# bentotten/radiation_ppo

Measured on AMD Instinct MI355X. Metric: env steps/sec (whole node) at 4096 envs; PPO iters/sec at 1/2/4/8 GPUs, higher is better.
Workload: dtype f32 policy / f64+int32 env

## Files before the change

radiation_ppo_amd/csrc/rs_ppo_grad2.hpp:

```cpp
#pragma once
#include "rs_mlp.hpp"

#define RS_T2 33

#ifdef RS_K7_STAMPS
#define RS_K7_NPH 16
__device__ unsigned long long rs_k7_stamp_table[2][RS_K7_NPH];
#define RS_STAMP_ENTRY const unsigned long long st_rt0 = __builtin_amdgcn_s_memrealtime(); const unsigned long long st_t0 = rs_k7_now();
#define RS_STAMP_DECL unsigned long long st_acc[RS_K7_NPH] = {0}; unsigned long long st_last = rs_k7_now(); st_acc[12] = st_last - st_t0;
#define RS_STAMP_EXIT(net) do { RS_STAMP(13); if ((threadIdx.x & 63) == 0) { st_acc[14] = __builtin_amdgcn_s_memrealtime() - st_rt0; \
                           for (int q = 0; q < RS_K7_NPH; ++q) atomicAdd(&rs_k7_stamp_table[net][q], st_acc[q]); } } while (0)
#define RS_STAMP(i) do { __builtin_amdgcn_sched_barrier(0); asm volatile("; RS_STAMP_MARK " #i); const unsigned long long t_ = rs_k7_now(); st_acc[i] += t_ - st_last; st_last = t_; \
                         __builtin_amdgcn_sched_barrier(0); } while (0)
__device__ __forceinline__ unsigned long long rs_k7_now() {
    unsigned long long t;
    asm volatile("s_memtime %0\n\ts_waitcnt lgkmcnt(0)" : "=s"(t) :: "memory");
    return t;
}
#else
#define RS_STAMP_ENTRY
#define RS_STAMP_DECL
#define RS_STAMP_EXIT(net)
#ifdef RS_K7_NO_PHASE_FENCE
#define RS_STAMP(i) do {} while (0)
#else
#define RS_STAMP(i) __builtin_amdgcn_sched_barrier(0)
#endif
#endif
#define RS_XRAW 400
#define RS_XSC 192
#define RS_G2_WAVE_FLOATS ((64 + 32) * RS_T2 + RS_XRAW + RS_XSC + 64)

__host__ __device__ constexpr int rs_grad2_lds_floats(int nout) {
    return ((rs_mlp_lds_floats(nout) + 3) & ~3) + 2 * 2 * 16 * 64 + 2 * 4 * 64 + 8 * RS_G2_WAVE_FLOATS;
}

__device__ __forceinline__ float rs_other_half(float x, int h) {
    const auto r = __builtin_amdgcn_permlane32_swap(__float_as_uint(x), __float_as_uint(x), false, false);
    return __uint_as_float(h ? r[0] : r[1]);
}

__device__ __forceinline__ void rs_stage32(float* T, const f32x16& v, int c, int h) {
#pragma unroll
    for (int r = 0; r < 16; ++r) T[rs_kappa(r, h) * RS_T2 + c] = v[r];
}

template <int NOUT>
__device__ __forceinline__ void rs_ppo_grad2_body(const RsMlpParams prm, const rs_ppo_batch B, float* partial,
                                                  double* stat_partial, const int* stop,
                                                  const rs_update_state* ust, int* snap,
                                                  const int bid, const int nblocks) {
    extern __shared__ __align__(16) float smem_f[];
    if (snap && bid == 0 && threadIdx.x == 0) { snap[0] = ust->adam_step; snap[1] = ust->stopped; }
    if (stop && *stop) return;
    RS_STAMP_ENTRY
    RsMlpLds<NOUT> W;
    W.carve(smem_f);
    float* w2tf = smem_f + ((rs_mlp_lds_floats(NOUT) + 3) & ~3);
    float* w3tf = w2tf + 2 * 2 * 16 * 64;
    const int wid = __builtin_amdgcn_readfirstlane(threadIdx.x >> 6);
    const int lane = threadIdx.x & 63, h = lane >> 5, c = lane & 31;
    const int l15 = lane & 15, l4 = lane >> 4;
    float* Qt = w3tf + 2 * 4 * 64 + wid * RS_G2_WAVE_FLOATS;
    float* Pt = Qt + 64 * RS_T2;
    float* xraw = Pt + 32 * RS_T2;
    float* xsc = xraw + RS_XRAW;
    float* dbl = xsc + RS_XSC;
    float* w1b = W.w1f;
    for (int i = threadIdx.x; i < 2 * 6 * 64; i += blockDim.x) {
        const int l = i & 63, s = (i >> 6) % 6, it = i / (6 * 64);
        const int row = 32 * it + (l & 31), k = 2 * s + (l >> 5);
        w1b[i] = RS_TANH_PRESCALE * ((k < RS_IN) ? prm.w1[row * RS_IN + k] : prm.b1[row]);
    }
    for (int i = threadIdx.x; i < 2 * 2 * 16 * 64; i += blockDim.x) {
        const int ri = i & 3, l = (i >> 2) & 63, r4 = (i >> 8) & 3, kt = (i >> 10) & 1, it = i >> 11;
        const int r = 4 * r4 + ri;
        w2tf[i] = prm.w2[(32 * kt + rs_kappa(r, l >> 5)) * RS_HID + 32 * it + (l & 31)];
        W.w2f[i] = RS_TANH_PRESCALE * prm.w2[(32 * it + (l & 31)) * RS_HID + 32 * kt + rs_kappa(r, l >> 5)];
    }
    for (int i = threadIdx.x; i < 2 * 4 * 64; i += blockDim.x) {
        int l = i & 63, sq = (i >> 6) & 3, it = i >> 8;
        int o = 2 * sq + (l >> 5);
        w3tf[i] = (o < NOUT) ? prm.w3[o * RS_HID + 32 * it + (l & 31)] : 0.0f;
    }
    for (int i = threadIdx.x; i < 2 * NOUT * 32; i += blockDim.x) {
        int q = i & 31, o = (i >> 5) % NOUT, hh = i / (32 * NOUT);
        if constexpr (NOUT == 8) { q = 4 * (i >> 6) + (i & 3); o = (i >> 2) & 7; hh = (i >> 5) & 1; }
        W.w3h[i] = prm.w3[o * RS_HID + 32 * (q >> 4) + rs_kappa(q & 15, hh)];
    }
    for (int i = threadIdx.x; i < 64; i += blockDim.x) W.b2[i] = RS_TANH_PRESCALE * prm.b2[i];
    for (int i = threadIdx.x; i < NOUT; i += blockDim.x) W.b3[i] = prm.b3[i];
    dbl[lane] = 0.0f;
    __syncthreads();

    const int M = B.M;
    const int groups = (M + 31) / 32;
    const int wave_g = bid * 8 + wid, n_waves = nblocks * 8;

    f32x16 acc2[2][2];
    f32x4 acc1[4], acc3[4];
#pragma unroll
    for (int a = 0; a < 2; ++a)
#pragma unroll
        for (int r = 0; r < 16; ++r) { acc2[a][0][r] = 0.f; acc2[a][1][r] = 0.f; }
#pragma unroll
    for (int a = 0; a < 4; ++a)
#pragma unroll
        for (int r = 0; r < 4; ++r) { acc1[a][r] = 0.f; acc3[a][r] = 0.f; }
    f32x4 accs;
#pragma unroll
    for (int r = 0; r < 4; ++r) accs[r] = 0.f;

    const int trips = (groups + n_waves - 1) / n_waves;
    const long x_last = (long)M * RS_IN - 1;
    auto dma_rows = [&](int g) {
        const char* gx = reinterpret_cast<const char*>(B.x + (long)g * (32 * RS_IN));
        const int lim = (int)(x_last - (long)g * (32 * RS_IN));
#pragma unroll
        for (int i = 0; i < 6; ++i) {
            const int o = min(i * 64 + lane, lim);
            __builtin_amdgcn_global_load_lds((const __attribute__((address_space(1))) void*)(gx + 4u * (unsigned)o),
                                             (__attribute__((address_space(3))) void*)(xraw + i * 64), 4, 0, 0);
        }
    };
    auto dma_scal = [&](int g) {
        const int m0 = g * 32;
        const int ms = min(m0 + c, M - 1);
        if constexpr (NOUT == 8) {
            const int mi = min(m0 + (lane >> 1), M - 1);
            const int* src = reinterpret_cast<const int*>(B.act) + 2 * (size_t)mi + (lane & 1);
            __builtin_amdgcn_global_load_lds((const __attribute__((address_space(1))) void*)src,
                                             (__attribute__((address_space(3))) void*)(xsc), 4, 0, 0);
        }
        if constexpr (NOUT == 8) {
            const float* src = (h ? B.logp_old : B.adv) + ms;
            __builtin_amdgcn_global_load_lds((const __attribute__((address_space(1))) void*)src,
                                             (__attribute__((address_space(3))) void*)(xsc + 64), 4, 0, 0);
        }
        {
            const float* src = (h ? B.ret : B.w) + ms;
            __builtin_amdgcn_global_load_lds((const __attribute__((address_space(1))) void*)src,
                                             (__attribute__((address_space(3))) void*)(xsc + 128), 4, 0, 0);
        }
    };
    {
        const int g0 = wave_g < groups ? wave_g : groups - 1;
        dma_rows(g0);
        dma_scal(g0);
    }
    float w3v[NOUT == 1 ? 32 : 1], db2r[2] = {0.0f, 0.0f};
    if constexpr (NOUT == 1) {
        const float4* wrow = reinterpret_cast<const float4*>(W.w3h + h * 32);
#pragma unroll
        for (int b = 0; b < 8; ++b) {
            const float4 t = wrow[b];
            w3v[4 * b + 0] = t.x; w3v[4 * b + 1] = t.y; w3v[4 * b + 2] = t.z; w3v[4 * b + 3] = t.w;
        }
    }
    RS_STAMP_DECL
    for (int trip = 0; trip < trips; ++trip) {
        RS_STAMP(15);
        const int gi_raw = wave_g + trip * n_waves;
        const int gi = gi_raw < groups ? gi_raw : groups - 1;
        const int m = gi * 32 + c;
        const bool valid = gi_raw < groups && m < M;
        asm volatile("s_waitcnt vmcnt(0)" ::: "memory");
#if defined(RS_K7_ALIGN) && RS_K7_ALIGN >= 1
        __builtin_amdgcn_s_barrier();
#endif
        const float wi = valid ? xsc[128 + c] : 0.0f;
        const int s_act = reinterpret_cast<const int*>(xsc)[2 * c];
        const float s_adv = xsc[64 + c], s_lpo = xsc[96 + c], s_ret = xsc[160 + c];
        float xv[6];
#pragma unroll
        for (int s6 = 0; s6 < 6; ++s6) xv[s6] = xraw[c * RS_IN + 2 * s6 + h];
        if (h) xv[5] = 1.0f;
        RS_STAMP(0);
        f32x16 H1[2], H2[2];
#pragma unroll
        for (int it = 0; it < 2; ++it)
#pragma unroll
            for (int r = 0; r < 16; ++r) H1[it][r] = 0.0f;
        {
            float a0 = w1b[(0 * 6 + 0) * 64 + lane], a1 = w1b[(1 * 6 + 0) * 64 + lane];
#pragma unroll
            for (int s = 0; s < 6; ++s) {
                const float b = xv[s];
                float n0 = 0.f, n1 = 0.f;
                if (s + 1 < 6) { n0 = w1b[(0 * 6 + s + 1) * 64 + lane]; n1 = w1b[(1 * 6 + s + 1) * 64 + lane]; }
                H1[0] = __builtin_amdgcn_mfma_f32_32x32x2f32(a0, b, H1[0], 0, 0, 0);
                H1[1] = __builtin_amdgcn_mfma_f32_32x32x2f32(a1, b, H1[1], 0, 0, 0);
                a0 = n0; a1 = n1;
            }
        }
        RS_STAMP(1);
#pragma unroll
        for (int it = 0; it < 2; ++it)
#pragma unroll
            for (int r = 0; r < 16; ++r) H1[it][r] = rs_tanh_scaled(H1[it][r]);
#pragma unroll
        for (int it = 0; it < 2; ++it)
#pragma unroll
            for (int q = 0; q < 4; ++q) {
                const float4 b = *reinterpret_cast<const float4*>(W.b2 + 32 * it + 8 * q + 4 * h);
                H2[it][4 * q + 0] = b.x; H2[it][4 * q + 1] = b.y; H2[it][4 * q + 2] = b.z; H2[it][4 * q + 3] = b.w;
            }
        RS_STAMP(2);
        {
            const float4* wq = reinterpret_cast<const float4*>(W.w2f) + lane;
            float4 a0 = wq[0], a1 = wq[(1 * 2 + 0) * 4 * 64];
#pragma unroll
            for (int g4 = 0; g4 < 8; ++g4) {
                const int kt = g4 >> 2, r0 = 4 * (g4 & 3);
                float4 n0 = a0, n1 = a1;
                if (g4 + 1 < 8) {
                    n0 = wq[((0 * 2 + ((g4 + 1) >> 2)) * 4 + ((g4 + 1) & 3)) * 64];
                    n1 = wq[((1 * 2 + ((g4 + 1) >> 2)) * 4 + ((g4 + 1) & 3)) * 64];
                }
                H2[0] = __builtin_amdgcn_mfma_f32_32x32x2f32(a0.x, H1[kt][r0 + 0], H2[0], 0, 0, 0);
                H2[1] = __builtin_amdgcn_mfma_f32_32x32x2f32(a1.x, H1[kt][r0 + 0], H2[1], 0, 0, 0);
                H2[0] = __builtin_amdgcn_mfma_f32_32x32x2f32(a0.y, H1[kt][r0 + 1], H2[0], 0, 0, 0);
                H2[1] = __builtin_amdgcn_mfma_f32_32x32x2f32(a1.y, H1[kt][r0 + 1], H2[1], 0, 0, 0);
                H2[0] = __builtin_amdgcn_mfma_f32_32x32x2f32(a0.z, H1[kt][r0 + 2], H2[0], 0, 0, 0);
                H2[1] = __builtin_amdgcn_mfma_f32_32x32x2f32(a1.z, H1[kt][r0 + 2], H2[1], 0, 0, 0);
                H2[0] = __builtin_amdgcn_mfma_f32_32x32x2f32(a0.w, H1[kt][r0 + 3], H2[0], 0, 0, 0);
                H2[1] = __builtin_amdgcn_mfma_f32_32x32x2f32(a1.w, H1[kt][r0 + 3], H2[1], 0, 0, 0);
                a0 = n0; a1 = n1;
            }
        }
        rs_stage32(Qt, H1[0], c, h);
        rs_stage32(Qt + 32 * RS_T2, H1[1], c, h);
        RS_STAMP(3);
#if defined(RS_K7_ALIGN) && RS_K7_ALIGN >= 2
        __builtin_amdgcn_s_barrier();
#endif
#pragma unroll
        for (int it = 0; it < 2; ++it)
#pragma unroll
            for (int r = 0; r < 16; ++r) H2[it][r] = rs_tanh_scaled(H2[it][r]);
        RS_STAMP(4);
        float out[NOUT];
        if constexpr (NOUT == 1) {
            float pacc = 0.0f;
#pragma unroll
            for (int q = 0; q < 32; ++q) pacc = fmaf(w3v[q], H2[q >> 4][q & 15], pacc);
            const float q = rs_other_half(pacc, h);
            out[0] = (h ? (q + pacc) : (pacc + q)) + W.b3[0];
        } else {
            f32x4 pacc[2];
#pragma unroll
            for (int r = 0; r < 4; ++r) { pacc[0][r] = 0.0f; pacc[1][r] = 0.0f; }
            const float4* wrow = reinterpret_cast<const float4*>(W.w3h) + 8 * h + (lane & 3);
            float4 wv[8][2];
#pragma unroll
            for (int b = 0; b < 8; ++b) { wv[b][0] = wrow[16 * b]; wv[b][1] = wrow[16 * b + 4]; }
#pragma unroll
            for (int b = 0; b < 8; ++b) {
                const int kt = b >> 2, r4 = b & 3;
                pacc[0] = __builtin_amdgcn_mfma_f32_4x4x1f32(wv[b][0].x, H2[kt][4 * r4 + 0], pacc[0], 0, 0, 0);
                pacc[1] = __builtin_amdgcn_mfma_f32_4x4x1f32(wv[b][1].x, H2[kt][4 * r4 + 0], pacc[1], 0, 0, 0);
                pacc[0] = __builtin_amdgcn_mfma_f32_4x4x1f32(wv[b][0].y, H2[kt][4 * r4 + 1], pacc[0], 0, 0, 0);
                pacc[1] = __builtin_amdgcn_mfma_f32_4x4x1f32(wv[b][1].y, H2[kt][4 * r4 + 1], pacc[1], 0, 0, 0);
                pacc[0] = __builtin_amdgcn_mfma_f32_4x4x1f32(wv[b][0].z, H2[kt][4 * r4 + 2], pacc[0], 0, 0, 0);
                pacc[1] = __builtin_amdgcn_mfma_f32_4x4x1f32(wv[b][1].z, H2[kt][4 * r4 + 2], pacc[1], 0, 0, 0);
                pacc[0] = __builtin_amdgcn_mfma_f32_4x4x1f32(wv[b][0].w, H2[kt][4 * r4 + 3], pacc[0], 0, 0, 0);
                pacc[1] = __builtin_amdgcn_mfma_f32_4x4x1f32(wv[b][1].w, H2[kt][4 * r4 + 3], pacc[1], 0, 0, 0);
            }
#pragma unroll
            for (int o = 0; o < NOUT; ++o) {
                const float p = pacc[o >> 2][o & 3];
                const float q = rs_other_half(p, h);
                out[o] = (h ? (q + p) : (p + q)) + W.b3[o];
            }
        }
        RS_STAMP(5);
        float dz[NOUT], sq[4];
        if (NOUT == 8) {
            const int a = s_act;
            const float adv = s_adv, lpo = s_lpo;
            float mx = out[0];
#pragma unroll
            for (int j = 1; j < NOUT; ++j) mx = fmaxf(mx, out[j]);
            float se = 0.f;
#pragma unroll
            for (int j = 0; j < NOUT; ++j) se += __expf(out[j] - mx);
            const float lse = __logf(se);
            float lp[NOUT], pj[NOUT], ent = 0.f, logp = 0.f;
#pragma unroll
            for (int j = 0; j < NOUT; ++j) {
                lp[j] = (out[j] - mx) - lse;
                pj[j] = __expf(lp[j]);
                ent -= pj[j] * lp[j];
                logp = (a == j) ? lp[j] : logp;
            }
            const float ratio = __expf(logp - lpo);
            const float lo = 1.0f - B.clip_ratio, hi = 1.0f + B.clip_ratio;
            const float clipped = fminf(fmaxf(ratio, lo), hi);
            const float s1 = ratio * adv, s2 = clipped * adv;
            const float surr = fminf(s1, s2);
            const bool inside = ratio >= lo && ratio <= hi;
            const float dr = (inside || s1 < s2) ? adv : 0.0f;
            const float g_lp = -wi * dr * ratio;
#pragma unroll
            for (int j = 0; j < NOUT; ++j) dz[j] = g_lp * (((a == j) ? 1.0f : 0.0f) - pj[j]);
            sq[0] = wi * (lpo - logp);
            sq[1] = wi * ent;
            sq[2] = wi * ((ratio > hi || ratio < lo) ? 1.0f : 0.0f);
            sq[3] = wi * surr;
        } else {
            const float diff = out[0] - s_ret;
            dz[0] = 2.0f * B.vf_coef * wi * diff;
            sq[0] = wi * diff * diff; sq[1] = 0.f; sq[2] = 0.f; sq[3] = 0.f;
        }
        RS_STAMP(6);

        float* Dz = xraw;
        if constexpr (NOUT == 1) {
            constexpr int T4 = 36;
            float* zrow = xraw + 96;
            float* ones = xraw + 160;
            zrow[32 * h + c] = h ? sq[0] : dz[0];
            ones[c] = 1.0f;
            float4 av[8];
#pragma unroll
            for (int hf = 0; hf < 2; ++hf) {
                rs_wave_sync();
#pragma unroll
                for (int r = 0; r < 16; ++r) Pt[rs_kappa(r, h) * T4 + c] = H2[hf][r];
                rs_wave_sync();
                if (hf == 0) {
#pragma unroll
                    for (int q = 0; q < 8; ++q) av[q] = *reinterpret_cast<const float4*>(zrow + 32 * (lane & 1) + 4 * q);
                }
                const float* brow = (hf == 0 && h) ? ones : Pt + c * T4;
                float4 bv[8];
#pragma unroll
                for (int q = 0; q < 8; ++q) bv[q] = *reinterpret_cast<const float4*>(brow + 4 * q);
#pragma unroll
                for (int q = 0; q < 8; ++q) {
                    acc3[hf] = __builtin_amdgcn_mfma_f32_4x4x1f32(av[q].x, bv[q].x, acc3[hf], 0, 0, 0);
                    acc3[hf] = __builtin_amdgcn_mfma_f32_4x4x1f32(av[q].y, bv[q].y, acc3[hf], 0, 0, 0);
                    acc3[hf] = __builtin_amdgcn_mfma_f32_4x4x1f32(av[q].z, bv[q].z, acc3[hf], 0, 0, 0);
                    acc3[hf] = __builtin_amdgcn_mfma_f32_4x4x1f32(av[q].w, bv[q].w, acc3[hf], 0, 0, 0);
                }
            }
        } else {
        if (h == 0) {
#pragma unroll
            for (int o = 0; o < NOUT; ++o) Dz[o * RS_T2 + c] = dz[o];
        } else {
#pragma unroll
            for (int q = 0; q < 4; ++q) Dz[(8 + q) * RS_T2 + c] = sq[q];
        }
#pragma unroll
        for (int hf = 0; hf < 2; ++hf) {
            rs_wave_sync();
            rs_stage32(Pt, H2[hf], c, h);
            rs_wave_sync();
            const bool a_row = l15 < NOUT || (l15 >= 8 && l15 < 12);
            float a_c = a_row ? Dz[l15 * RS_T2 + l4] : 0.0f;
            float b_c[2];
#pragma unroll
            for (int u = 0; u < 2; ++u) b_c[u] = Pt[(16 * u + l15) * RS_T2 + l4];
#pragma unroll
            for (int s = 0; s < 8; ++s) {
                float a_n = 0.f, b_n[2] = {0.f, 0.f};
                if (s + 1 < 8) {
                    a_n = a_row ? Dz[l15 * RS_T2 + 4 * (s + 1) + l4] : 0.0f;
#pragma unroll
                    for (int u = 0; u < 2; ++u) b_n[u] = Pt[(16 * u + l15) * RS_T2 + 4 * (s + 1) + l4];
                }
                const float a_dz = (l15 < NOUT) ? a_c : 0.0f;
#pragma unroll
                for (int u = 0; u < 2; ++u) acc3[2 * hf + u] = __builtin_amdgcn_mfma_f32_16x16x4f32(a_dz, b_c[u], acc3[2 * hf + u], 0, 0, 0);
                if (hf == 0) accs = __builtin_amdgcn_mfma_f32_16x16x4f32(a_c, 1.0f, accs, 0, 0, 0);
                a_c = a_n;
#pragma unroll
                for (int u = 0; u < 2; ++u) b_c[u] = b_n[u];
            }
        }
        }
        RS_STAMP(7);
        if (NOUT == 8) {
#pragma unroll
            for (int it = 0; it < 2; ++it) {
                f32x16 t;
#pragma unroll
                for (int r = 0; r < 16; ++r) t[r] = 0.f;
#pragma unroll
                for (int s = 0; s < 4; ++s) {
                    const float b = h ? dz[(2 * s + 1) % NOUT] : dz[(2 * s) % NOUT];
                    t = __builtin_amdgcn_mfma_f32_32x32x2f32(w3tf[(it * 4 + s) * 64 + lane], b, t, 0, 0, 0);
                }
#pragma unroll
                for (int r = 0; r < 16; ++r) { const float hv = H2[it][r]; H2[it][r] = fmaf(-(t[r] * hv), hv, t[r]); }
            }
        } else {
#pragma unroll
            for (int kt = 0; kt < 2; ++kt)
#pragma unroll
                for (int r = 0; r < 16; ++r) {
                    const float hv = H2[kt][r];
                    const float d = w3v[kt * 16 + r] * dz[0];
                    H2[kt][r] = fmaf(-(d * hv), hv, d);
                }
        }
        {
            const int gn_raw = wave_g + (trip + 1) * n_waves;
            const int gn = gn_raw < groups ? gn_raw : groups - 1;
            asm volatile("s_waitcnt lgkmcnt(0)" ::: "memory");
            dma_rows(gn);
            dma_scal(gn);
        }
        RS_STAMP(8);
#if defined(RS_K7_ALIGN) && RS_K7_ALIGN >= 3
        __builtin_amdgcn_s_barrier();
#endif
        rs_wave_sync();
        rs_stage32(Pt, H2[0], c, h);
        f32x16 D1[2];
#pragma unroll
        for (int it = 0; it < 2; ++it)
#pragma unroll
            for (int r = 0; r < 16; ++r) D1[it][r] = 0.f;
        {
            const float4* wq = reinterpret_cast<const float4*>(w2tf) + lane;
            float4 a0 = wq[0], a1 = wq[(1 * 2 + 0) * 4 * 64];
#pragma unroll
            for (int g4 = 0; g4 < 8; ++g4) {
                const int kt = g4 >> 2, r0 = 4 * (g4 & 3);
                float4 n0 = a0, n1 = a1;
                if (g4 + 1 < 8) {
                    n0 = wq[((0 * 2 + ((g4 + 1) >> 2)) * 4 + ((g4 + 1) & 3)) * 64];
                    n1 = wq[((1 * 2 + ((g4 + 1) >> 2)) * 4 + ((g4 + 1) & 3)) * 64];
                }
                D1[0] = __builtin_amdgcn_mfma_f32_32x32x2f32(a0.x, H2[kt][r0 + 0], D1[0], 0, 0, 0);
                D1[1] = __builtin_amdgcn_mfma_f32_32x32x2f32(a1.x, H2[kt][r0 + 0], D1[1], 0, 0, 0);
                D1[0] = __builtin_amdgcn_mfma_f32_32x32x2f32(a0.y, H2[kt][r0 + 1], D1[0], 0, 0, 0);
                D1[1] = __builtin_amdgcn_mfma_f32_32x32x2f32(a1.y, H2[kt][r0 + 1], D1[1], 0, 0, 0);
                D1[0] = __builtin_amdgcn_mfma_f32_32x32x2f32(a0.z, H2[kt][r0 + 2], D1[0], 0, 0, 0);
                D1[1] = __builtin_amdgcn_mfma_f32_32x32x2f32(a1.z, H2[kt][r0 + 2], D1[1], 0, 0, 0);
                D1[0] = __builtin_amdgcn_mfma_f32_32x32x2f32(a0.w, H2[kt][r0 + 3], D1[0], 0, 0, 0);
                D1[1] = __builtin_amdgcn_mfma_f32_32x32x2f32(a1.w, H2[kt][r0 + 3], D1[1], 0, 0, 0);
                a0 = n0; a1 = n1;
            }
        }
        float xb[8];
        {
            int gi_late = gi;
            asm volatile("" : "+v"(gi_late));
#pragma unroll
            for (int s8 = 0; s8 < 8; ++s8) {
                int n = gi_late * 32 + 4 * s8 + l4;
                n = n < M ? n : M - 1;
                xb[s8] = (l15 < RS_IN) ? B.x[(size_t)n * RS_IN + l15] : ((l15 == RS_IN) ? 1.0f : 0.0f);
            }
        }
#pragma unroll
        for (int it = 0; it < 2; ++it)
#pragma unroll
            for (int r = 0; r < 16; ++r) {
                const float hv = Qt[(32 * it + rs_kappa(r, h)) * RS_T2 + c];
                const float d = D1[it][r];
                D1[it][r] = fmaf(-(d * hv), hv, d);
            }
        rs_wave_sync();
        RS_STAMP(9);
#pragma unroll
        for (int it = 0; it < 2; ++it) {
            if (it == 1) {
                rs_wave_sync();
                rs_stage32(Pt, H2[1], c, h);
                rs_wave_sync();
            }
            float a_c = Pt[c * RS_T2 + h], b0_c = Qt[c * RS_T2 + h], b1_c = Qt[(32 + c) * RS_T2 + h];
#pragma unroll
            for (int s = 0; s < 16; ++s) {
                float a_n = 0.f, b0_n = 0.f, b1_n = 0.f;
                if (s + 1 < 16) {
                    a_n = Pt[c * RS_T2 + 2 * (s + 1) + h];
                    b0_n = Qt[c * RS_T2 + 2 * (s + 1) + h];
                    b1_n = Qt[(32 + c) * RS_T2 + 2 * (s + 1) + h];
                }
                acc2[it][0] = __builtin_amdgcn_mfma_f32_32x32x2f32(a_c, b0_c, acc2[it][0], 0, 0, 0);
                acc2[it][1] = __builtin_amdgcn_mfma_f32_32x32x2f32(a_c, b1_c, acc2[it][1], 0, 0, 0);
                a_c = a_n; b0_c = b0_n; b1_c = b1_n;
            }
            float rs = 0.0f;
#pragma unroll
            for (int n = 0; n < 16; ++n) rs += Pt[c * RS_T2 + 16 * h + n];
            rs += rs_other_half(rs, h);
            if constexpr (NOUT == 1) db2r[it] += rs;
            else if (h == 0) dbl[32 * it + c] += rs;
        }
        RS_STAMP(10);
#pragma unroll
        for (int it = 0; it < 2; ++it) {
            rs_wave_sync();
            rs_stage32(Pt, D1[it], c, h);
            rs_wave_sync();
            float a0_c = Pt[l15 * RS_T2 + l4], a1_c = Pt[(16 + l15) * RS_T2 + l4];
#pragma unroll
            for (int s = 0; s < 8; ++s) {
                float a0_n = 0.f, a1_n = 0.f;
                if (s + 1 < 8) {
                    a0_n = Pt[l15 * RS_T2 + 4 * (s + 1) + l4];
                    a1_n = Pt[(16 + l15) * RS_T2 + 4 * (s + 1) + l4];
                }
                acc1[2 * it + 0] = __builtin_amdgcn_mfma_f32_16x16x4f32(a0_c, xb[s], acc1[2 * it + 0], 0, 0, 0);
                acc1[2 * it + 1] = __builtin_amdgcn_mfma_f32_16x16x4f32(a1_c, xb[s], acc1[2 * it + 1], 0, 0, 0);
                a0_c = a0_n; a1_c = a1_n;
            }
        }
        rs_wave_sync();
        RS_STAMP(11);
    }
    constexpr int RS_REST = rs_net_params(NOUT) - 64 * 64;
    static_assert(8 * 64 * 64 <= rs_grad2_lds_floats(NOUT) && 8 * ((RS_REST + 1) & ~1) + 2 * 8 * 5 <= rs_grad2_lds_floats(NOUT),
                  "the epilogue's slabs must fit K7's LDS");
    int tid_e = threadIdx.x;
    asm volatile("" : "+v"(tid_e));
    const int lane_e = tid_e & 63, h_e = lane_e >> 5, c_e = lane_e & 31, l15_e = lane_e & 15, l4_e = lane_e >> 4;
    asm volatile("s_waitcnt vmcnt(0)" ::: "memory");
    const float db2v = NOUT == 1 ? (h_e ? db2r[1] : db2r[0]) : dbl[lane_e];
    __syncthreads();
    float* outp = partial + (size_t)bid * rs_net_params(NOUT);
    {
        float* g_w2 = smem_f + wid * (64 * 64);
#pragma unroll
        for (int it = 0; it < 2; ++it)
#pragma unroll
            for (int r = 0; r < 16; ++r) {
                const int row = 32 * it + rs_kappa(r, h_e);
                g_w2[row * 64 + c_e] = acc2[it][0][r];
                g_w2[row * 64 + 32 + c_e] = acc2[it][1][r];
            }
    }
    __syncthreads();
    for (int i = tid_e; i < 64 * 64; i += blockDim.x) {
        float v = 0.0f + smem_f[i];
#pragma unroll
        for (int wv = 1; wv < 8; ++wv) v += smem_f[wv * (64 * 64) + i];
        outp[64 * RS_IN + 64 + i] = v;
    }
    float db3r[NOUT];
    double sv[5];
    if constexpr (NOUT == 1) {
        db3r[0] = __shfl(acc3[0][0], 32);
        sv[0] = 0.0; sv[1] = 0.0; sv[2] = 0.0; sv[3] = (double)__shfl(acc3[0][1], 32); sv[4] = 0.0;
    } else {
#pragma unroll
        for (int o = 0; o < NOUT; ++o) db3r[o] = __shfl(accs[o & 3], 16 * (o >> 2));
        const float t0 = __shfl(accs[0], 32), t1 = __shfl(accs[1], 32), t2 = __shfl(accs[2], 32), t3 = __shfl(accs[3], 32);
        sv[0] = (double)t0; sv[1] = (double)t1; sv[2] = (double)t2; sv[3] = 0.0; sv[4] = (double)t3;
    }
    constexpr int RS_RSTR = (RS_REST + 1) & ~1;
    double* sred = reinterpret_cast<double*>(smem_f + 8 * RS_RSTR);
    __syncthreads();
    {
        float* g_w1 = smem_f + wid * RS_RSTR, *g_b1 = g_w1 + 64 * RS_IN, *g_b2 = g_b1 + 64, *g_w3 = g_b2 + 64, *g_b3 = g_w3 + NOUT * 64;
        g_b2[lane_e] = db2v;
#pragma unroll
        for (int u = 0; u < 4; ++u)
#pragma unroll
            for (int q = 0; q < 4; ++q) {
                const int row = 16 * u + 4 * l4_e + q;
                if (l15_e < RS_IN) g_w1[row * RS_IN + l15_e] = acc1[u][q];
                if (l15_e == RS_IN) g_b1[row] = acc1[u][q];
                const int o = 4 * l4_e + q;
                if (NOUT == 8 && o < NOUT) g_w3[o * 64 + 16 * u + l15_e] = acc3[u][q];
            }
        if (NOUT == 1 && lane_e < 32) { g_w3[lane_e] = acc3[0][0]; g_w3[32 + lane_e] = acc3[1][0]; }
        if (lane_e == 0) {
#pragma unroll
            for (int o = 0; o < NOUT; ++o) g_b3[o] = db3r[o];
#pragma unroll
            for (int q = 0; q < 5; ++q) sred[wid * 5 + q] = sv[q];
        }
    }
    __syncthreads();
    for (int i = tid_e; i < RS_REST; i += blockDim.x) {
        float v = 0.0f + smem_f[i];
#pragma unroll
        for (int wv = 1; wv < 8; ++wv) v += smem_f[wv * RS_RSTR + i];
        outp[i < 64 * RS_IN + 64 ? i : i + 64 * 64] = v;
    }
    if (tid_e < 5) {
        double v = 0.0 + sred[tid_e];
#pragma unroll
        for (int wv = 1; wv < 8; ++wv) v += sred[wv * 5 + tid_e];
        stat_partial[(size_t)bid * 5 + tid_e] = v;
    }
    RS_STAMP_EXIT(NOUT == 8 ? 0 : 1);
}

template <int NOUT>
__global__ void __launch_bounds__(512, 2) rs_ppo_grad2_kernel(RsMlpParams prm, rs_ppo_batch B, float* __restrict__ partial,
                                                              double* __restrict__ stat_partial, const int* __restrict__ stop,
                                                              const rs_update_state* __restrict__ ust, int* __restrict__ snap) {
    rs_ppo_grad2_body<NOUT>(prm, B, partial, stat_partial, stop, ust, snap, blockIdx.x, gridDim.x);
}

__global__ void __launch_bounds__(512, 2) rs_ppo_grad2_pair_kernel(RsMlpParams pa, RsMlpParams pc, rs_ppo_batch B, float* __restrict__ partial_a,
                                                                   float* __restrict__ partial_c, double* __restrict__ stat_a,
                                                                   double* __restrict__ stat_c, const int* __restrict__ stop,
                                                                   const rs_update_state* __restrict__ ust, int* __restrict__ snap) {
    const int G = gridDim.x >> 1;
    if ((int)blockIdx.x < G) rs_ppo_grad2_body<8>(pa, B, partial_a, stat_a, stop, nullptr, nullptr, blockIdx.x, G);
    else rs_ppo_grad2_body<1>(pc, B, partial_c, stat_c, stop, ust, snap, blockIdx.x - G, G);
}
```

Before: 42.23 million.

## Use 4x4x1 MFMA blocks for w3 gradient and pack tanh math into float2

Replaces the 16x16x4 MFMA outer product for the NOUT=8 w3/b3 gradient with 4x4x1 multi-block MFMAs. It reads a padded (stride 36) transposed tile with float4 LDS loads, which cuts the wasted zero rows and the shuffled scalar LDS reads. The tanh forward and the tanh-derivative loops are rewritten as two-wide vector ops so the compiler can emit packed FMA/mul. The accumulator layout, the shuffle indices for db3/stats and the w3 gradient writeback change to match the new MFMA output mapping. This relies on layout reasoning being correct and on the padded tile fitting inside the xraw/xsc scratch.

```diff
diff --git a/radiation_ppo_amd/csrc/rs_ppo_grad2.hpp b/radiation_ppo_amd/csrc/rs_ppo_grad2.hpp
--- a/radiation_ppo_amd/csrc/rs_ppo_grad2.hpp
+++ b/radiation_ppo_amd/csrc/rs_ppo_grad2.hpp
@@ -39,6 +39,20 @@
     const auto r = __builtin_amdgcn_permlane32_swap(__float_as_uint(x), __float_as_uint(x), false, false);
     return __uint_as_float(h ? r[0] : r[1]);
 }
+
+typedef float rs_f2 __attribute__((ext_vector_type(2)));
+
+__device__ __forceinline__ void rs_tanh_scaled16(f32x16& v) {
+#pragma unroll
+    for (int r = 0; r < 16; r += 2) {
+        const rs_f2 e = (rs_f2){1.0f, 1.0f} + (rs_f2){__builtin_amdgcn_exp2f(v[r]), __builtin_amdgcn_exp2f(v[r + 1])};
+        const rs_f2 t = __builtin_elementwise_fma((rs_f2){-2.0f, -2.0f}, (rs_f2){__builtin_amdgcn_rcpf(e.x), __builtin_amdgcn_rcpf(e.y)},
+                                                  (rs_f2){1.0f, 1.0f});
+        v[r] = t.x; v[r + 1] = t.y;
+    }
+}
+
+__device__ __forceinline__ rs_f2 rs_dtanh2(rs_f2 d, rs_f2 hv) { return __builtin_elementwise_fma(-(d * hv), hv, d); }
 
 __device__ __forceinline__ void rs_stage32(float* T, const f32x16& v, int c, int h) {
 #pragma unroll
@@ -98,15 +112,17 @@
     const int wave_g = bid * 8 + wid, n_waves = nblocks * 8;
 
     f32x16 acc2[2][2];
-    f32x4 acc1[4], acc3[4];
+    f32x4 acc1[4], acc3[2];
 #pragma unroll
     for (int a = 0; a < 2; ++a)
 #pragma unroll
         for (int r = 0; r < 16; ++r) { acc2[a][0][r] = 0.f; acc2[a][1][r] = 0.f; }
 #pragma unroll
-    for (int a = 0; a < 4; ++a)
-#pragma unroll
-        for (int r = 0; r < 4; ++r) { acc1[a][r] = 0.f; acc3[a][r] = 0.f; }
+    for (int r = 0; r < 4; ++r) {
+#pragma unroll
+        for (int a = 0; a < 4; ++a) acc1[a][r] = 0.f;
+        acc3[0][r] = 0.f; acc3[1][r] = 0.f;
+    }
     f32x4 accs;
 #pragma unroll
     for (int r = 0; r < 4; ++r) accs[r] = 0.f;
@@ -196,8 +212,7 @@
         RS_STAMP(1);
 #pragma unroll
         for (int it = 0; it < 2; ++it)
-#pragma unroll
-            for (int r = 0; r < 16; ++r) H1[it][r] = rs_tanh_scaled(H1[it][r]);
+            rs_tanh_scaled16(H1[it]);
 #pragma unroll
         for (int it = 0; it < 2; ++it)
 #pragma unroll
@@ -236,8 +251,7 @@
 #endif
 #pragma unroll
         for (int it = 0; it < 2; ++it)
-#pragma unroll
-            for (int r = 0; r < 16; ++r) H2[it][r] = rs_tanh_scaled(H2[it][r]);
+            rs_tanh_scaled16(H2[it]);
         RS_STAMP(4);
         float out[NOUT];
         if constexpr (NOUT == 1) {
@@ -314,7 +328,6 @@
         }
         RS_STAMP(6);
 
-        float* Dz = xraw;
         if constexpr (NOUT == 1) {
             constexpr int T4 = 36;
             float* zrow = xraw + 96;
@@ -345,40 +358,43 @@
                 }
             }
         } else {
-        if (h == 0) {
-#pragma unroll
-            for (int o = 0; o < NOUT; ++o) Dz[o * RS_T2 + c] = dz[o];
-        } else {
-#pragma unroll
-            for (int q = 0; q < 4; ++q) Dz[(8 + q) * RS_T2 + c] = sq[q];
-        }
-#pragma unroll
-        for (int hf = 0; hf < 2; ++hf) {
-            rs_wave_sync();
-            rs_stage32(Pt, H2[hf], c, h);
-            rs_wave_sync();
-            const bool a_row = l15 < NOUT || (l15 >= 8 && l15 < 12);
-            float a_c = a_row ? Dz[l15 * RS_T2 + l4] : 0.0f;
-            float b_c[2];
-#pragma unroll
-            for (int u = 0; u < 2; ++u) b_c[u] = Pt[(16 * u + l15) * RS_T2 + l4];
-#pragma unroll
-            for (int s = 0; s < 8; ++s) {
-                float a_n = 0.f, b_n[2] = {0.f, 0.f};
-                if (s + 1 < 8) {
-                    a_n = a_row ? Dz[l15 * RS_T2 + 4 * (s + 1) + l4] : 0.0f;
-#pragma unroll
-                    for (int u = 0; u < 2; ++u) b_n[u] = Pt[(16 * u + l15) * RS_T2 + 4 * (s + 1) + l4];
-                }
-                const float a_dz = (l15 < NOUT) ? a_c : 0.0f;
-#pragma unroll
-                for (int u = 0; u < 2; ++u) acc3[2 * hf + u] = __builtin_amdgcn_mfma_f32_16x16x4f32(a_dz, b_c[u], acc3[2 * hf + u], 0, 0, 0);
-                if (hf == 0) accs = __builtin_amdgcn_mfma_f32_16x16x4f32(a_c, 1.0f, accs, 0, 0, 0);
-                a_c = a_n;
-#pragma unroll
-                for (int u = 0; u < 2; ++u) b_c[u] = b_n[u];
-            }
-        }
+            constexpr int T4 = 36;
+            float* Az = xraw + 96;
+            static_assert(32 * T4 == 32 * RS_T2 + 96 && 96 + 12 * T4 <= RS_XRAW + RS_XSC, "h2^T tile and A rows end inside xraw + xsc");
+#pragma unroll
+            for (int o = 0; o < NOUT; ++o) Az[o * T4 + c] = dz[o];
+#pragma unroll
+            for (int q = 0; q < 4; ++q) Az[(8 + q) * T4 + c] = sq[q];
+            const float* arow = Az + (lane & 7) * T4;
+            const float* srow = Az + min(l15, 11) * T4;
+            const float* brow = Pt + (4 * (lane >> 3) + (lane & 3)) * T4;
+            float4 av[8];
+#pragma unroll
+            for (int hf = 0; hf < 2; ++hf) {
+                rs_wave_sync();
+#pragma unroll
+                for (int r = 0; r < 16; ++r) Pt[rs_kappa(r, h) * T4 + c] = H2[hf][r];
+                rs_wave_sync();
+                if (hf == 0) {
+#pragma unroll
+                    for (int q = 0; q < 8; ++q) av[q] = *reinterpret_cast<const float4*>(arow + 4 * q);
+                }
+                float4 bv[8], zv[4];
+#pragma unroll
+                for (int q = 0; q < 4; ++q) zv[q] = *reinterpret_cast<const float4*>(srow + 16 * hf + 4 * q);
+#pragma unroll
+                for (int q = 0; q < 8; ++q) bv[q] = *reinterpret_cast<const float4*>(brow + 4 * q);
+#pragma unroll
+                for (int q = 0; q < 8; ++q) {
+                    const float z0 = (q & 1) ? zv[q >> 1].z : zv[q >> 1].x, z1 = (q & 1) ? zv[q >> 1].w : zv[q >> 1].y;
+                    acc3[hf] = __builtin_amdgcn_mfma_f32_4x4x1f32(av[q].x, bv[q].x, acc3[hf], 0, 0, 0);
+                    accs = __builtin_amdgcn_mfma_f32_4x4x1f32(z0, 1.0f, accs, 0, 0, 0);
+                    acc3[hf] = __builtin_amdgcn_mfma_f32_4x4x1f32(av[q].y, bv[q].y, acc3[hf], 0, 0, 0);
+                    acc3[hf] = __builtin_amdgcn_mfma_f32_4x4x1f32(av[q].z, bv[q].z, acc3[hf], 0, 0, 0);
+                    accs = __builtin_amdgcn_mfma_f32_4x4x1f32(z1, 1.0f, accs, 0, 0, 0);
+                    acc3[hf] = __builtin_amdgcn_mfma_f32_4x4x1f32(av[q].w, bv[q].w, acc3[hf], 0, 0, 0);
+                }
+            }
         }
         RS_STAMP(7);
         if (NOUT == 8) {
@@ -393,16 +409,19 @@
                     t = __builtin_amdgcn_mfma_f32_32x32x2f32(w3tf[(it * 4 + s) * 64 + lane], b, t, 0, 0, 0);
                 }
 #pragma unroll
-                for (int r = 0; r < 16; ++r) { const float hv = H2[it][r]; H2[it][r] = fmaf(-(t[r] * hv), hv, t[r]); }
+                for (int r = 0; r < 16; r += 2) {
+                    const rs_f2 d = rs_dtanh2((rs_f2){t[r], t[r + 1]}, (rs_f2){H2[it][r], H2[it][r + 1]});
+                    H2[it][r] = d.x; H2[it][r + 1] = d.y;
+                }
             }
         } else {
 #pragma unroll
             for (int kt = 0; kt < 2; ++kt)
 #pragma unroll
-                for (int r = 0; r < 16; ++r) {
-                    const float hv = H2[kt][r];
-                    const float d = w3v[kt * 16 + r] * dz[0];
-                    H2[kt][r] = fmaf(-(d * hv), hv, d);
+                for (int r = 0; r < 16; r += 2) {
+                    const rs_f2 d = (rs_f2){w3v[kt * 16 + r], w3v[kt * 16 + r + 1]} * (rs_f2){dz[0], dz[0]};
+                    const rs_f2 e = rs_dtanh2(d, (rs_f2){H2[kt][r], H2[kt][r + 1]});
+                    H2[kt][r] = e.x; H2[kt][r + 1] = e.y;
                 }
         }
         {
@@ -459,10 +478,10 @@
 #pragma unroll
         for (int it = 0; it < 2; ++it)
 #pragma unroll
-            for (int r = 0; r < 16; ++r) {
-                const float hv = Qt[(32 * it + rs_kappa(r, h)) * RS_T2 + c];
-                const float d = D1[it][r];
-                D1[it][r] = fmaf(-(d * hv), hv, d);
+            for (int r = 0; r < 16; r += 2) {
+                const rs_f2 hv = {Qt[(32 * it + rs_kappa(r, h)) * RS_T2 + c], Qt[(32 * it + rs_kappa(r + 1, h)) * RS_T2 + c]};
+                const rs_f2 d = rs_dtanh2((rs_f2){D1[it][r], D1[it][r + 1]}, hv);
+                D1[it][r] = d.x; D1[it][r + 1] = d.y;
             }
         rs_wave_sync();
         RS_STAMP(9);
@@ -550,8 +569,8 @@
         sv[0] = 0.0; sv[1] = 0.0; sv[2] = 0.0; sv[3] = (double)__shfl(acc3[0][1], 32); sv[4] = 0.0;
     } else {
 #pragma unroll
-        for (int o = 0; o < NOUT; ++o) db3r[o] = __shfl(accs[o & 3], 16 * (o >> 2));
-        const float t0 = __shfl(accs[0], 32), t1 = __shfl(accs[1], 32), t2 = __shfl(accs[2], 32), t3 = __shfl(accs[3], 32);
+        for (int o = 0; o < NOUT; ++o) db3r[o] = __shfl(accs[o & 3], 4 * (o >> 2));
+        const float t0 = __shfl(accs[0], 8), t1 = __shfl(accs[1], 8), t2 = __shfl(accs[2], 8), t3 = __shfl(accs[3], 8);
         sv[0] = (double)t0; sv[1] = (double)t1; sv[2] = (double)t2; sv[3] = 0.0; sv[4] = (double)t3;
     }
     constexpr int RS_RSTR = (RS_REST + 1) & ~1;
@@ -567,9 +586,14 @@
                 const int row = 16 * u + 4 * l4_e + q;
                 if (l15_e < RS_IN) g_w1[row * RS_IN + l15_e] = acc1[u][q];
                 if (l15_e == RS_IN) g_b1[row] = acc1[u][q];
-                const int o = 4 * l4_e + q;
-                if (NOUT == 8 && o < NOUT) g_w3[o * 64 + 16 * u + l15_e] = acc3[u][q];
-            }
+            }
+        if constexpr (NOUT == 8) {
+#pragma unroll
+            for (int hf = 0; hf < 2; ++hf)
+#pragma unroll
+                for (int i = 0; i < 4; ++i)
+                    g_w3[(4 * ((lane_e >> 2) & 1) + i) * 64 + 32 * hf + 4 * (lane_e >> 3) + (lane_e & 3)] = acc3[hf][i];
+        }
         if (NOUT == 1 && lane_e < 32) { g_w3[lane_e] = acc3[0][0]; g_w3[32 + lane_e] = acc3[1][0]; }
         if (lane_e == 0) {
 #pragma unroll
```

After: 43.03 million, median of 6. +1.9%, better.
